# DixianZhu/deBWT

Measured on AMD Instinct MI355X. Metric: Gbp/sec BWT build (30 Gbp synthetic DNA); bit-exact vs CPU ref; 1/2/4/8-GPU, higher is better.
Workload: dtype u64

## Files before the change

### debwt_amd/_lib.py

```python
import ctypes
import os
import subprocess

_HERE = os.path.dirname(os.path.abspath(__file__))
LIB_PATH = os.environ.get("DEBWT_HIP_LIB", os.path.join(_HERE, "libdebwt_hip.so"))
_lib = None


class DebwtConfig(ctypes.Structure):
    _fields_ = [("k", ctypes.c_int), ("device", ctypes.c_int), ("sort_algo", ctypes.c_int),
                ("reserved", ctypes.c_int)]


class DebwtPackedText(ctypes.Structure):
    _fields_ = [("words", ctypes.POINTER(ctypes.c_uint64)), ("nwords", ctypes.c_uint64), ("n", ctypes.c_uint64),
                ("sep", ctypes.POINTER(ctypes.c_uint64)), ("nrec", ctypes.c_uint64),
                ("seconds_read", ctypes.c_double), ("seconds_pack", ctypes.c_double)]


class DebwtStats(ctypes.Structure):
    _fields_ = ([(n, ctypes.c_uint64) for n in (
        "n", "nrec", "red_capacity", "blue_capacity", "blue_bound_num", "case3num", "sp_len",
        "special_branch_num", "n_main", "distinct_keys", "blue_large_blocks", "blue_max_block")] +
        [(n, ctypes.c_float) for n in (
            "ms_extract", "ms_sort", "ms_classify", "ms_sp", "ms_blue", "ms_assemble", "ms_total",
            "ms_host_special")] +
        [("radix_pass_launches", ctypes.c_uint32), ("radix_pass_ms", ctypes.c_float),
         ("radix_pass_keys", ctypes.c_uint64), ("special_path", ctypes.c_uint32), ("special_threads", ctypes.c_uint32),
         ("sort_unfit_stretches", ctypes.c_uint64), ("sort_unfit_network", ctypes.c_uint64),
         ("sort_over_stretches", ctypes.c_uint64), ("sort_bucket_passes", ctypes.c_uint64)])

    def as_dict(self):
        return {n: getattr(self, n) for n, _ in self._fields_}


class DebwtVerifyReport(ctypes.Structure):
    _fields_ = ([(n, ctypes.c_uint64) for n in ("segments", "steps", "mismatches", "broken_links", "search_failures",
                                                "search_steps")] +
                [(n, ctypes.c_float) for n in ("ms_index", "ms_search", "ms_walk")] + [("ok", ctypes.c_int)])

    def as_dict(self):
        return {n: getattr(self, n) for n, _ in self._fields_}


MULTI_STEPS = 24


class DebwtShardReport(ctypes.Structure):
    _fields_ = [("ms", ctypes.c_float * MULTI_STEPS), ("bytes_in", ctypes.c_uint64 * 5), ("bytes_out", ctypes.c_uint64 * 5),
                ("keys", ctypes.c_uint64), ("key_ranges", ctypes.c_uint64), ("blocks", ctypes.c_uint64),
                ("blue_rows", ctypes.c_uint64), ("rows", ctypes.c_uint64), ("bin_lo", ctypes.c_uint32), ("bin_hi", ctypes.c_uint32)]


class DebwtFmInfo(ctypes.Structure):
    _fields_ = ([(n, ctypes.c_uint64) for n in ("n", "nrec", "sa_sample", "samples", "device_bytes")] +
                [("ms_rank", ctypes.c_float), ("ms_samples", ctypes.c_float), ("census", ctypes.c_uint64 * 4)])

    def as_dict(self):
        d = {n: getattr(self, n) for n, _ in self._fields_}
        d["census"] = [int(x) for x in self.census]
        return d


# ... 690 lines not shown
```

### debwt_amd/csrc/debwt_hip.hip

```cpp
#include "../../include/debwt_hip.h"

#include <hip/hip_runtime.h>

#include <algorithm>
#include <new>
#include <chrono>
#include <cmath>
#include <cstdio>
#include <cstring>
#include <atomic>
#include <string>
#include <thread>
#include <tuple>
#include <vector>

#include "radix_sort.h"
#include "special_host.h"
#include "fasta_host.h"
#include "gz_parallel.h"
#include "stage_kernels.h"
#include "special_kernels.h"
#include "verify_kernels.h"
#include "fm_kernels.h"
#include "fm_search_kernels.h"
// ... 804 lines not shown
                    (unsigned long long)r.M, (unsigned long long)in_heavy, (unsigned)RS_BUCKET_HEAVY, (unsigned long long)largest,
                    r.heavy ? "four HBM passes" : "bucket pass");
    }
    return DEBWT_OK;
}

static int sort_begin(debwt_ctx *c) {
    const u64 n = c->n;
    if (c->stage > ST_LOADED) c->stage = ST_LOADED;
    int rc = plan_ranges(c);
    if (rc) return rc;
    u64 maxM = 0;
    for (auto &r : c->ranges) maxM = std::max(maxM, r.M);
    struct ReclaimScope { debwt_ctx *c; ~ReclaimScope() { c->reclaim_ok = false; } } rscope{c};
    c->reclaim_ok = true;
    if (!c->exchange) ENSURE(c, c->keysA, maxM * 8 + 64);
    ENSURE(c, c->keysB, maxM * 8 + 64);
    ENSURE(c, c->rs_skew, (maxM / 2048 + 2) * 4);
    ENSURE(c, c->rs_rle, radix_rle_ws_bytes(maxM));
    if ((rc = heavy_ranges(c))) return rc;
    size_t pair_bytes = 0;
    for (auto &r : c->ranges) {
        const u64 range[2] = {r.key_lo, r.key_hi};
        pair_bytes = std::max(pair_bytes, radix_pair_bytes_u64(r.M, 2 * c->cfg.k, range, r.heavy));
    }
    ENSURE(c, c->rs_pair, pair_bytes);
    ENSURE(c, c->dk, maxM * 8 + 64);
    ENSURE(c, c->dstart, maxM * 4 + 64);
    ENSURE(c, c->pflag, maxM + 64);
    ENSURE(c, c->mchar, c->Mctx + 64);
    c->reclaim_ok = false;
    c->Q = c->B = c->nlarge = 0; c->nfacts_acc = 0; c->n1024 = 0; c->n512 = 0; c->Dsum = 0;
    c->st.sort_unfit_stretches = c->st.sort_unfit_network = c->st.sort_over_stretches = c->st.sort_bucket_passes = 0;
    const size_t P = c->ranges.size();
    HIPCHK(c, hipEventRecord(c->ev[0], c->stream));
    HIPCHK(c, hipEventRecord(c->ev[1], c->stream));
    join_special(c);
    c->special_dev = false;
    if (special_wants_device(c)) {
        if ((rc = special_device_build(c))) return rc;
    } else {
    c->special_running = true;
    c->special_thread = std::thread([c, n]() {
        auto t0 = std::chrono::steady_clock::now();
        build_special_tables(c->h_text, n, c->h_sep.data(), c->nrec, c->K, &c->special);
        c->st.ms_host_special = std::chrono::duration<float, std::milli>(std::chrono::steady_clock::now() - t0).count();
        c->st.special_threads = c->special.threads_used;
        c->st.special_path = c->special.threads_used > 1 ? 1 : 0;
    });
    }
    c->shared_hist = P <= RS_MAX_RANGES && !c->exchange &&
                     (P > 1 || (P == 1 && n >= (1ull << 26) && range_split(c, c->ranges[0]).hbm_shift > 0));
    if (c->shared_hist) {
        const int kb = 2 * c->cfg.k;
        std::vector<u8> rob(SHARD_BINS, 0xFF);
        int shifts[RS_MAX_RANGES];
        for (size_t i = 0; i < P; i++) {
            const u32 lo = (u32)(c->ranges[i].key_lo >> (kb - 12));
            const u32 hi = c->ranges[i].key_hi ? (u32)(c->ranges[i].key_hi >> (kb - 12)) : SHARD_BINS;
            for (u32 b = lo; b < hi; b++) rob[b] = (u8)i;
            shifts[i] = range_split(c, c->ranges[i]).hbm_shift;
        }
        ENSURE(c, c->dest_tab, SHARD_BINS);
        ENSURE(c, c->range_hist, P * radix_text_hist_stride() * sizeof(u32));
        HIPCHK(c, hipMemcpyAsync(c->dest_tab.p, rob.data(), SHARD_BINS, hipMemcpyHostToDevice, c->stream));
        TextKeySrc all{c->text.as<u64>(), c->sepbits.as<u64>(), n, c->K, 0, 0, 0, nullptr, nullptr, 0};
// ... 31 lines not shown
    if (i == 0 && !c->special_dev) {
        join_special(c);
        const SpecialTables &sp = c->special;
        c->nbranch = sp.branch.size();
        ENSURE(c, c->branch, sp.branch.size() * 8 + 64);
        HIPCHK(c, hipMemcpyAsync(c->head_keys.p, sp.head_keys.data(), c->nrec * 8, hipMemcpyHostToDevice, c->stream));
        HIPCHK(c, hipMemcpyAsync(c->spkey.p, sp.key.data(), c->NS * 8, hipMemcpyHostToDevice, c->stream));
        HIPCHK(c, hipMemcpyAsync(c->spchr.p, sp.chr.data(), c->NS, hipMemcpyHostToDevice, c->stream));
        if (!sp.branch.empty())
            HIPCHK(c, hipMemcpyAsync(c->branch.p, sp.branch.data(), sp.branch.size() * 8, hipMemcpyHostToDevice, c->stream));
        if ((rc = special_branch_bitmap(c))) return rc;
    }
    u64 *d_bounds = nullptr;
    {
        const std::vector<uint64_t> &key = c->special.key;
        u64 s0 = 0, s1 = c->NS;
        if ((c->shard_world > 1 || P > 1) && c->special_dev) {
            d_bounds = c->dollar.as<u64>() + 5;
            k_sp_bounds<<<1, 64, 0, c->stream>>>(c->spkey.as<u64>(), c->NS, r.key_lo >> 2, r.key_hi >> 2, d_bounds);
            HIPCHK(c, hipMemcpyAsync(&c->h_scalars[24], d_bounds, 16, hipMemcpyDeviceToHost, c->stream));
        } else if (c->shard_world > 1 || P > 1) {
            s0 = std::lower_bound(key.begin(), key.end(), r.key_lo >> 2) - key.begin();
            s1 = r.key_hi ? (u64)(std::lower_bound(key.begin(), key.end(), r.key_hi >> 2) - key.begin()) : c->NS;
        }
        r.s0 = s0; r.s1 = s1;
    }
    if ((rc = sync_check(c))) return rc;
    if (d_bounds) memcpy(&r.s0, &c->h_scalars[24], 8), memcpy(&r.s1, &c->h_scalars[26], 8);
    c->D = c->h_scalars[0];
    c->Dsum += c->D;
    if (sink.done) {
        c->st.sort_unfit_stretches += c->h_scalars[32]; c->st.sort_unfit_network += c->h_scalars[35];
        c->st.sort_over_stretches += sink.n_over;
    }
    if (r.s1 > r.s0)
        k_special_rows<<<grid_for(r.s1 - r.s0, 256), 256, 0, c->stream>>>(
            c->dk.as<u64>(), c->dstart.as<u32>(), c->D, r.M, c->spkey.as<u64>() + r.s0, r.s1 - r.s0,
            r.Mbase + (r.s0 - c->ranges[0].s0), c->sprow.as<u64>() + r.s0);
    if (P > 1 || c->exchange) {
        if ((rc = classify_local(c))) return rc;
        if ((rc = append_range(c, r))) return rc;
    }
    return DEBWT_OK;
}

static int sort_end(debwt_ctx *c) {
    c->s0 = c->ranges.front().s0; c->s1 = c->ranges.back().s1;
    if (c->ranges.size() > 1 || c->exchange) {
        c->local_done = true;
        HIPCHK(c, hipEventRecord(c->ev[2], c->stream));
        HIPCHK(c, hipEventRecord(c->ev[3], c->stream));
    }
    c->st.distinct_keys = c->Dsum;
    c->st.special_branch_num = c->nbranch;
    c->stage = ST_SORTED;
    return DEBWT_OK;
}

extern "C" int debwt_kmer_sort_rle(debwt_ctx *c) {
    if (!c) return DEBWT_EINVAL;
    if (c->stage < ST_LOADED) return DEBWT_ESTATE;
    if (c->exchange) { c->err = "exchange-mode shard: use debwt_shard_sort_begin/_range/_end"; return DEBWT_ESTATE; }
    HIPCHK(c, hipSetDevice(c->cfg.device));
    int rc = sort_begin(c);
    for (size_t i = 0; !rc && i < c->ranges.size(); i++) rc = sort_range(c, i, nullptr);
    join_special(c);
// ... 6343 lines not shown
```

### debwt_amd/csrc/radix_sort.hip

```cpp
#include "radix_sort.h"

#include <algorithm>
#include <atomic>
#include <cstddef>
#include <utility>
#include <cstdio>
#include <cstdlib>
#include <vector>


template <int FIXED0>
__device__ __forceinline__ u32 rs_digit(const RsDigit &g, u64 k) {
    if (FIXED0 == 2) return __builtin_amdgcn_ubfe((u32)(k >> 32), (u32)g.shift - 32u, (u32)__popc(g.mask));
    if (FIXED0 || g.mode == 0) {
        const u32 lo = (u32)k, hi = (u32)(k >> 32);
        const bool up = g.shift >= 32;
        return __builtin_amdgcn_alignbit(up ? 0u : hi, up ? hi : lo, (u32)g.shift & 31u) & g.mask;
    }
    if (g.mode == 1) return g.tab[(k >> g.tshift) & 4095u];
    u32 q = (u32)(k >> g.tshift), lo = 0, hi = g.nb;
    if (hi <= 16u) {
        for (u32 i = 1; i < hi; i++) lo += g.bounds[i] <= q ? 1u : 0u;
        return lo;
    }
// ... 1526 lines not shown
        for (int r = 0; r < KPT; r++)
            if (cr[r] != 0xFFFFFFFFu) A[RL_PAD(cr[r])] = kk[r];
        __syncthreads();
        if (!tcnt) {
            for (u32 j = tid; j < cnt; j += NT) keys[s + j] = A[RL_PAD(j)];
        } else {
            for (u32 j = tid; j < cnt; j += NT) mchar[s + j] = (u8)(A[RL_PAD(j)] & 3ull);
            u32 hm = 0;
            u64 prev = tid ? A[RL_PAD(tid * KPT - 1)] : 0ull;
#pragma unroll
            for (int r = 0; r < KPT; r++) {
                const u32 j = tid * KPT + (u32)r;
                const u64 key = A[RL_PAD(j)];
                hm |= ((j < cnt && (j == 0 || key != prev)) ? 1u : 0u) << r;
                prev = key;
            }
            const u32 cl = (u32)__popc(hm);
            u32 c;
            u32 o = block_scan_excl(cl, wtmp, &c);
            const bool staged = stg != nullptr && RLT_STAGE_RATIO * c <= cnt;
            if (tid == 0) { tcnt[t] = c | (staged ? RLT_STAGED : 0u); unfit[i] = t | RLU_COUNTED; }
            if (staged) {
                u64 *kd = stg + s;
                unsigned short *id = reinterpret_cast<unsigned short *>(stg + s + c);
#pragma unroll
                for (int r = 0; r < KPT; r++)
                    if ((hm >> r) & 1u) { kd[o] = A[RL_PAD(tid * KPT + r)]; id[o] = (unsigned short)(tid * KPT + r); o++; }
            }
            if (!(staged && drop_sorted))
                for (u32 j = tid; j < cnt; j += NT) keys[s + j] = A[RL_PAD(j)];
        }
    }
}
#endif

__global__ __launch_bounds__(256) void rs_local_unfit_net_kernel(u64 *__restrict__ keys, u64 n, const u64 *__restrict__ bnd,
                                                                 u32 nwtiles, u32 *__restrict__ unfit,
                                                                 const u32 *__restrict__ nunfit, u32 *__restrict__ over,
                                                                 u32 over_cap) {
    constexpr int KPT = 16, NT = 256;
    constexpr u32 CAP = NT * KPT;
    __shared__ u64 A[CAP + CAP / 16];
    const u32 tid = threadIdx.x;
    const u32 nu = nunfit[0];
    if (RLU_CLASSIFY && nunfit[3] == 0) return;
    for (u32 i = blockIdx.x; i < nu; i += gridDim.x) {
        u32 t = unfit[i];
        if (RLU_CLASSIFY) {
            if (!(t & RLU_NET_FLAG)) continue;
            t &= ~RLU_NET_FLAG;
            __syncthreads();
            if (tid == 0) unfit[i] = t;
        }
        const u64 s = bnd[t], e = t + 1 < nwtiles ? bnd[t + 1] : n;
        const u64 cnt64 = e - s;
        __syncthreads();
        if (cnt64 > CAP) {
            if (RLU_CLASSIFY) continue;
            u32 bad = 0;
            for (u64 j = s + tid; j + 1 < e && !bad; j += NT) bad = keys[j] > keys[j + 1] ? 1u : 0u;
            if (__syncthreads_or((int)bad) && tid == 0) {
                const u32 idx = atomicAdd(&over[0], 1u);
                if (idx < over_cap) {
                    u64 *list = reinterpret_cast<u64 *>(over + 4);
                    list[2 * idx] = s; list[2 * idx + 1] = cnt64;
                }
// ... 202 lines not shown
            const u32 m = l_n;
            for (u32 q = 0; q < m; q++) {
                const u32 t = l_t[q];
                const u64 s = l_s[q], e = l_e[q];
                const u32 K = (u32)((e - (u64)t * RLW_H) / RLW_H);
                const u64 k0 = (u64)gy + (W + G - t % G) % G;
                if (k0 >= K) continue;
                const u64 kfirst = keys[s];
                const bool one_run = kfirst == keys[e - 1];
                for (u64 k = k0; k < K; k += G) piece(t, s, e, K, (u32)k, kfirst, one_run);
            }
        }
        return;
    }
    for (u32 i = blockIdx.x; i < nu; i += gridDim.x) {
        const u32 entry = unfit[i];
        const u32 t = RLU_TILE(entry);
        if (entry & RLU_COUNTED) {
            if (!EMIT || ((tcnt[t] & RLT_STAGED) && staging_ok)) continue;
        }
        const u64 s = bnd[t], e = t + 1 < nwtiles ? bnd[t + 1] : n;
        const u64 K64 = (e - (u64)t * RLW_H) / RLW_H;
        const u32 K = (K64 < 1 || (entry & RLU_COUNTED)) ? 1u : (u32)K64;
        if (K >= RLU_LONG) continue;
        const u64 kfirst = keys[s];
        const bool one_run = kfirst == keys[e - 1];
        for (u32 k = 0; k < K; k++) piece(t, s, e, K, k, kfirst, one_run);
    }
}


static size_t rle_nw(u64 n) { return (size_t)(n / RLW_H + 2); }
static size_t rle_nb(u64 n) { return rle_nw(n) / RLT_BLOCK + 2; }
size_t radix_rle_ws_bytes(u64 n) { return 16 + rle_nw(n) * (8 + 12) + rle_nb(n) * 8 + 64; }

__global__ __launch_bounds__(256) void rs_over_move(u64 *__restrict__ keys, u64 *__restrict__ scratch, const u64 *__restrict__ list,
                                                    const u64 *__restrict__ offs, u32 nranges, u64 total, int back,
                                                    const u64 *__restrict__ base = nullptr, int W = 0) {
    const u64 g0 = (u64)blockIdx.x * 1024u;
    if (g0 >= total) return;
    u32 lo = 0, hi = nranges;
    while (lo + 1 < hi) { u32 mid = (lo + hi) >> 1; if (offs[mid] <= g0) lo = mid; else hi = mid; }
    const u64 wmask = W ? (1ull << W) - 1ull : 0ull;
#pragma unroll
    for (int j = 0; j < 4; j++) {
        const u64 g = g0 + (u64)j * 256u + threadIdx.x;
        if (g >= total) break;
        u32 r = lo;
        while (r + 1 < nranges && offs[r + 1] <= g) r++;
        const u64 src = list[2 * r] + (g - offs[r]);
        if (!base) { if (back) keys[src] = scratch[g]; else scratch[g] = keys[src]; }
        else if (back) keys[src] = (scratch[g] & wmask) + base[r];
        else scratch[g] = ((u64)r << W) | (keys[src] - base[r]);
    }
}
__global__ void rs_over_ends(const u64 *__restrict__ keys, const u64 *__restrict__ list, u32 nranges, u64 *__restrict__ ends) {
    const u32 r = blockIdx.x * blockDim.x + threadIdx.x;
    if (r >= nranges) return;
    ends[2 * r] = keys[list[2 * r]];
    ends[2 * r + 1] = keys[list[2 * r] + list[2 * r + 1] - 1];
}

#define RB_NT 256
#define RB_KPT 16
#define RB_CAP (RB_NT * RB_KPT)
#define RB_H (4 * RB_CAP)
#define RB_UNROLL 4
// ... 255 lines not shown
        if (ev) (void)hipEventRecord(pass_events[2 * ev_idx], stream);
        if (aux && strip_last && shift + bits >= hi_bit) {
            dg.out_strip = strip_last;
            rs_scatter_kernel<0, 2, 0><<<nchunks, SC_NT, 0, stream>>>(src, none, dst, n, chunk, dg, ws.counts, digit_tot, nchunks, ctab);
        } else if (aux) rs_scatter_kernel<0, 1, 0><<<nchunks, SC_NT, 0, stream>>>(src, none, dst, n, chunk, dg, ws.counts, digit_tot, nchunks, ctab);
        else if (shift >= 32) rs_scatter_kernel<0, 0, 1><<<nchunks, SC_NT, 0, stream>>>(src, none, dst, n, chunk, dg, ws.counts, digit_tot, nchunks, ctab);
        else rs_scatter_kernel<0, 0, 0><<<nchunks, SC_NT, 0, stream>>>(src, none, dst, n, chunk, dg, ws.counts, digit_tot, nchunks, ctab);
        if (ev) { (void)hipEventRecord(pass_events[2 * ev_idx + 1], stream); ev_idx++; if (npairs) *npairs = ev_idx; }
        derived = pp.nv != 0;
        if (derived) {
            rs_pair_bounds_kernel<<<(nchunks + 1 + 255) / 256, 256, 0, stream>>>(ws.counts, digit_tot, nchunks, pp.rows, n, chunk, nchunks, pair_tab);
            rs_pair_derive_kernel<<<nchunks, RS_RADIX, 0, stream>>>(pair_J, pair_tab, pp.nv, pp.vbase, ws.counts, nchunks);
            rs_pair_launched.fetch_add(1, std::memory_order_relaxed);
        }
        if (final_dst) { src = dst; dst = (npasses - (p + 2)) % 2 == 0 ? final_dst : (src == a ? third : a); }
        else if (third) { src = dst; dst = p + 2 == npasses ? a : (src == b ? third : b); }
        else { u64 *t = src; src = dst; dst = t; }
    }
    return src;
}

size_t radix_text_hist_stride() { return (size_t)RS_RADIX * RS_MAXCHUNKS; }

static int rs_bucket_mode() {
    const char *e = getenv("DEBWT_BUCKET_PASS");
    return !e || !*e ? -1 : (atoi(e) != 0 ? 1 : 0);
}

static int rs_forced_digits() {
    const char *e = getenv("DEBWT_PREFIX_DIGITS");
    const int t = e && *e ? atoi(e) : 0;
    return t >= 1 && t <= 4 ? t : 0;
}
static bool rs_finish_low() {
    const char *e = getenv("DEBWT_FINISH_LOW");
    return !e || !*e || atoi(e) != 0;
}

RadixSplit radix_split(u64 n, int key_bits, int algo, const u64 *range, bool heavy) {
    algo &= 15;
    if (key_bits > 64) key_bits = 64;
    const int mode = rs_bucket_mode();
    int T = 0;
    while ((n >> (8 * T)) > RS_BUCKET_TARGET && T < 4) T++;
    if (mode == 1 && T < 2) T = 2;
    if (rs_forced_digits()) T = rs_forced_digits();
    RadixSplit sp{false, false, 0, 0, 0};
    if (algo != 3 || T == 0 || key_bits - 8 * T < 1) return sp;
    sp.hybrid = true;
    sp.T = T;
    sp.pshift = key_bits - 8 * T;
    const bool ranged = range && (range[0] || range[1]);
    sp.bucket = mode == 1 ? T >= 2 : (mode != 0 && T == 4 && ranged && !heavy);
    sp.hbm_shift = sp.bucket ? sp.pshift + 8 : sp.pshift;
    return sp;
}

static std::atomic<u64> rs_bucket_launched{0};
u64 radix_bucket_passes() { return rs_bucket_launched.load(std::memory_order_relaxed); }
static std::atomic<u64> rs_low_finishes{0};
u64 radix_low_finishes() { return rs_low_finishes.load(std::memory_order_relaxed); }

hipError_t radix_text_hist_ranges(hipStream_t stream, const TextKeySrc &text, const u8 *range_of_bin, int key_bits,
                                  const int *shift, int nranges, u32 *counts) {
    if (nranges < 1 || nranges > RS_MAX_RANGES) return hipErrorInvalidValue;
    u32 nchunks; u64 chunk;
// ... 48 lines not shown
    const bool net_only = (algo & 32) != 0;
    (void)net_only;
    algo &= 15;
    if (key_bits > 64) key_bits = 64;
    if (!text && (n < (rs_bucket_mode() == 1 ? 1u : 2u) || key_bits <= 0)) return a;
    const u64 text_range[2] = {text ? text->key_lo : 0ull, text ? text->key_hi : 0ull};
    if (!key_range && text) key_range = text_range;
    const RadixSplit sp = radix_split(n, key_bits, algo, key_range, heavy);
    if (!sp.hybrid || !ws.over || !ws.h_over) {
        u64 *r = rs_lsd(stream, a, b, n, 0, key_bits, ws, pass_events, max_pairs, npairs, text, aux, 0, nullptr, nullptr, key_range);
        *err = hipGetLastError();
        return r;
    }
    const int pshift = sp.pshift;
    u64 *src = rs_lsd(stream, a, b, n, sp.hbm_shift, key_bits, ws, pass_events, max_pairs, npairs, text, aux, 0, nullptr, nullptr, key_range);
    u64 *other = src == a ? b : a;
    if (sp.bucket && n > 0) {
        const u32 nbt = (u32)((n + RB_H - 1) / RB_H);
        rs_bucket_digit_kernel<<<nbt, RB_NT, 0, stream>>>(src, other, n, sp.hbm_shift, pshift);
        rs_bucket_launched.fetch_add(1, std::memory_order_relaxed);
        u64 *t = src; src = other; other = t;
    }
    const bool low = pshift <= 32 && rs_finish_low();
    if (low) rs_low_finishes.fetch_add(1, std::memory_order_relaxed);
    (void)hipMemsetAsync(ws.over, 0, 16, stream);
    u32 ntiles = (u32)((n + RL_H - 1) / RL_H), nwtiles = (u32)((n + RLW_H - 1) / RLW_H);
    u8 *mark = reinterpret_cast<u8 *>(ws.skew_list);
    (void)hipMemsetAsync(mark, 0, ntiles + 1, stream);
    u32 *rle_ctr = nullptr, *rle_tcnt = nullptr, *rle_unfit = nullptr, *rle_tex = nullptr, *rle_bsum = nullptr, *rle_boff = nullptr;
    u64 *rle_bnd = nullptr;
    if (sink) {
        const size_t nw = rle_nw(n);
        rle_ctr = static_cast<u32 *>(sink->ws);
        rle_bnd = reinterpret_cast<u64 *>(rle_ctr + 4);
        rle_tcnt = reinterpret_cast<u32 *>(rle_bnd + nw);
        rle_unfit = rle_tcnt + nw;
        rle_tex = rle_unfit + nw;
        rle_bsum = rle_tex + nw;
        rle_boff = rle_bsum + rle_nb(n);
        (void)hipMemsetAsync(rle_ctr, 0, 16, stream);
        if (low)
            rs_local_count_kernel<true><<<nwtiles, 64, 0, stream>>>(src, n, pshift, mark, rle_bnd, rle_unfit, rle_ctr, rle_tcnt, sink->mchar,
                                                                    sink->no_staging ? nullptr : other, sink->drop_sorted ? 1 : 0);
        else
            rs_local_count_kernel<false><<<nwtiles, 64, 0, stream>>>(src, n, pshift, mark, rle_bnd, rle_unfit, rle_ctr, rle_tcnt, sink->mchar,
                                                                     sink->no_staging ? nullptr : other, sink->drop_sorted ? 1 : 0);
        const u32 ugrid = nwtiles < 16384u ? nwtiles : 16384u;
#if RLU_CLASSIFY
        u64 *const stg = sink->no_staging ? nullptr : other;
        rs_local_unfit_kernel<8><<<ugrid, 256, 0, stream>>>(src, n, rle_bnd, nwtiles, rle_unfit, rle_ctr, ws.over, ws.over_cap,
                                                            net_only ? 0u : RLU_GAP_MAX, rle_tcnt, sink->mchar, stg, sink->drop_sorted ? 1 : 0);
        rs_local_unfit_kernel<16><<<ugrid < 4096u ? ugrid : 4096u, 256, 0, stream>>>(src, n, rle_bnd, nwtiles, rle_unfit, rle_ctr, ws.over,
                                                                                      ws.over_cap, net_only ? 0u : RLU_GAP_MAX,
                                                                                      rle_tcnt, sink->mchar, stg, sink->drop_sorted ? 1 : 0);
#endif
        rs_local_unfit_net_kernel<<<ugrid, 256, 0, stream>>>(src, n, rle_bnd, nwtiles, rle_unfit, rle_ctr, ws.over, ws.over_cap);
    } else {
        if (low) rs_local_kernel<64, true><<<nwtiles, 64, 0, stream>>>(src, n, pshift, ws.over, ws.over_cap, mark);
        else rs_local_kernel<64><<<nwtiles, 64, 0, stream>>>(src, n, pshift, ws.over, ws.over_cap, mark);
        rs_local_kernel<256><<<ntiles, 256, 0, stream>>>(src, n, pshift, ws.over, ws.over_cap, mark);
    }
    (void)hipMemcpyAsync(ws.h_over, ws.over, 16, hipMemcpyDeviceToHost, stream);
    if ((*err = hipStreamSynchronize(stream)) != hipSuccess) return src;
    u32 nover = ws.h_over[0];
    bool staging_lost = false;
    if (nover) {
        bool whole = nover > ws.over_cap;
        u64 total = 0;
        std::vector<u64> offs, hlist;
        if (!whole) {
            hlist.resize(2 * (size_t)nover);
            (void)hipMemcpyAsync(hlist.data(), ws.over + 4, 16 * (size_t)nover, hipMemcpyDeviceToHost, stream);
            if ((*err = hipStreamSynchronize(stream)) != hipSuccess) return src;
            const u64 *list = hlist.data();
            std::vector<std::pair<u64, u64>> rg(nover);
            for (u32 i = 0; i < nover; i++) rg[i] = {list[2 * i], list[2 * i + 1]};
            std::sort(rg.begin(), rg.end());
            offs.resize(3 * (size_t)nover);
            for (u32 i = 0; i < nover; i++) {
                offs[i] = total; total += rg[i].second;
                offs[nover + 2 * i] = rg[i].first; offs[nover + 2 * i + 1] = rg[i].second;
            }
// ... 39 lines not shown
                    dmax = std::max(dmax, (ends[2 * i + 1] >> pshift) - (ends[2 * i] >> pshift));
                }
                int wb = pshift, rb = 1;
                while (wb < 64 && (dmax >> (wb - pshift))) wb++;
                while ((1ull << rb) < nover) rb++;
                if (wb + rb <= key_bits - 8) {
                    (void)hipMemcpyAsync(d_base, base.data(), 8 * (size_t)nover, hipMemcpyHostToDevice, stream);
                    if ((*err = hipStreamSynchronize(stream)) != hipSuccess) return src;
                    cbase = d_base; W = wb; sort_bits = wb + rb;
                }
            }
            rs_over_move<<<grid, 256, 0, stream>>>(src, scratch, d_list, d_offs, nover, total, 0, cbase, W);
            u64 *r = rs_lsd(stream, scratch, tmp, total, 0, sort_bits, ws, nullptr, 0, nullptr, nullptr, true);
            rs_over_move<<<grid, 256, 0, stream>>>(src, r, d_list, d_offs, nover, total, 1, cbase, W);
            if ((*err = hipStreamSynchronize(stream)) != hipSuccess) return src;
        }
    }
    if (sink) {
        const u32 ug = nwtiles < 2048u ? nwtiles : 2048u;
        const u32 nb = (nwtiles + RLT_BLOCK - 1) / RLT_BLOCK;
        rs_unfit_rle_kernel<0, 0><<<ug, 256, 0, stream>>>(src, n, rle_bnd, nwtiles, rle_unfit, rle_ctr, rle_tcnt, rle_tex,
                                                       rle_boff, sink->dk, sink->dstart, sink->mchar, staging_lost ? 0 : 1);
                rs_unfit_rle_kernel<0, 1><<<dim3(64, RLU_ROWS), RLU_LONG_NT, 0, stream>>>(src, n, rle_bnd, nwtiles, rle_unfit, rle_ctr, rle_tcnt, rle_tex,
                                                       rle_boff, sink->dk, sink->dstart, sink->mchar, staging_lost ? 0 : 1);
        rs_tile_scan1_kernel<<<nb, 256, 0, stream>>>(rle_tcnt, nwtiles, rle_tex, rle_bsum);
        rs_tile_scan2_kernel<<<1, 1024, 0, stream>>>(rle_bsum, nb, rle_boff, rle_ctr + 1);
        rs_tile_emit_kernel<<<(nwtiles + 3) / 4, 256, 0, stream>>>(src, n, rle_bnd, nwtiles, rle_tex, rle_boff, sink->dk, sink->dstart,
                                                                   rle_tcnt, staging_lost ? nullptr : other);
        rs_unfit_rle_kernel<1, 0><<<ug, 256, 0, stream>>>(src, n, rle_bnd, nwtiles, rle_unfit, rle_ctr, rle_tcnt, rle_tex,
                                                       rle_boff, sink->dk, sink->dstart, sink->mchar, staging_lost ? 0 : 1);
                rs_unfit_rle_kernel<1, 1><<<dim3(64, RLU_ROWS), RLU_LONG_NT, 0, stream>>>(src, n, rle_bnd, nwtiles, rle_unfit, rle_ctr, rle_tcnt, rle_tex,
                                                       rle_boff, sink->dk, sink->dstart, sink->mchar, staging_lost ? 0 : 1);
        (void)hipMemcpyAsync(sink->h_total, rle_ctr + 1, sizeof(u32), hipMemcpyDeviceToHost, stream);
        if (sink->h_ctr) (void)hipMemcpyAsync(sink->h_ctr, rle_ctr, 4 * sizeof(u32), hipMemcpyDeviceToHost, stream);
        sink->n_over = nover;
        sink->done = true;
    }
    *err = hipGetLastError();
    return src;
}

hipError_t radix_partition_by_shard(hipStream_t stream, const u64 *src, const TextKeySrc *text, u64 count, u64 *dst,
                                    const RsDigit &dg, u32 nshards, const RadixWorkspace &ws, u64 *offs_host, bool sparse,
                                    u64 capacity) {
    TextKeySrc none{};
    u32 nchunks; u64 chunk;
    rs_plan(count, &nchunks, &chunk);
    u32 *digit_tot = ws.counts + (size_t)RS_RADIX * RS_MAXCHUNKS;
    if (text) {
        TextKeySrc ts = *text;
        rs_hist_kernel<1, 1><<<nchunks, RS_BLOCK, 0, stream>>>(nullptr, ts, count, chunk, dg, ws.counts, nchunks);
    } else {
        rs_hist_kernel<0, 1><<<nchunks, RS_BLOCK, 0, stream>>>(src, none, count, chunk, dg, ws.counts, nchunks);
    }
    rs_scan_digit_kernel<<<RS_RADIX, 1024, 0, stream>>>(ws.counts, nchunks, digit_tot);
    rs_scan_tot_kernel<<<1, RS_RADIX, 0, stream>>>(digit_tot);
    u32 tot[RS_RADIX];
    hipError_t e = hipMemcpyAsync(tot, digit_tot, sizeof tot, hipMemcpyDeviceToHost, stream);
    if (e != hipSuccess) return e;
    if ((e = hipStreamSynchronize(stream)) != hipSuccess) return e;
    for (u32 i = 0; i < nshards; i++) offs_host[i] = tot[i];
    offs_host[nshards] = nshards < RS_RADIX ? tot[nshards] : 0;
    if (offs_host[nshards] > capacity) return hipErrorInvalidValue;
    if (text && sparse) rs_scatter_sparse_kernel<0, 1><<<nchunks, SC_NT, 0, stream>>>(*text, dst, count, chunk, dg, ws.counts, digit_tot, nchunks);
    else if (text) rs_scatter_kernel<1, 1, 0><<<nchunks, SC_NT, 0, stream>>>(nullptr, *text, dst, count, chunk, dg, ws.counts, digit_tot, nchunks);
    else rs_scatter_kernel<0, 1, 0><<<nchunks, SC_NT, 0, stream>>>(src, none, dst, count, chunk, dg, ws.counts, digit_tot, nchunks);
    if ((e = hipStreamSynchronize(stream)) != hipSuccess) return e;
// ... 3 lines not shown
```

### include/debwt_hip.h

```cpp
#ifndef DEBWT_HIP_H
#define DEBWT_HIP_H
#include <stddef.h>
#include <stdint.h>
#ifdef __cplusplus
extern "C" {
#endif

#define DEBWT_OK 0
#define DEBWT_EINVAL (-1)
#define DEBWT_ENOMEM (-2)
#define DEBWT_EDEVICE (-3)
#define DEBWT_ESTATE (-4)
#define DEBWT_ERANGE (-5)
#define DEBWT_EINTERNAL (-6)
#define DEBWT_EIO (-7)

typedef struct debwt_ctx debwt_ctx;

typedef struct {
    int k;
    int device;
    int sort_algo;
    int reserved;
} debwt_config;

typedef struct {
    uint64_t n;
    uint64_t nrec;
    uint64_t red_capacity;
    uint64_t blue_capacity;
    uint64_t blue_bound_num;
    uint64_t case3num;
    uint64_t sp_len;
    uint64_t special_branch_num;
    uint64_t n_main;
    uint64_t distinct_keys;
    uint64_t blue_large_blocks;
    uint64_t blue_max_block;
    float ms_extract, ms_sort, ms_classify, ms_sp, ms_blue, ms_assemble, ms_total, ms_host_special;
    uint32_t radix_pass_launches;
    float radix_pass_ms;
    uint64_t radix_pass_keys;
    uint32_t special_path, special_threads;
    uint64_t sort_unfit_stretches, sort_unfit_network, sort_over_stretches;
    uint64_t sort_bucket_passes;
} debwt_stats;

int debwt_create(const debwt_config *cfg, debwt_ctx **out);
void debwt_destroy(debwt_ctx *ctx);
const char *debwt_strerror(int code);
const char *debwt_last_error(const debwt_ctx *ctx);
int debwt_get_config(const debwt_ctx *ctx, debwt_config *out);

int debwt_load_text(debwt_ctx *ctx, const uint64_t *packed, uint64_t n, const uint64_t *sep, uint64_t nrec);

int debwt_load_ascii(debwt_ctx *ctx, const char *seq, const uint64_t *reclen, uint64_t nrec);

typedef struct {
    uint64_t *words;
    uint64_t nwords;
    uint64_t n;
    uint64_t *sep;
    uint64_t nrec;
    double seconds_read, seconds_pack;
} debwt_packed_text;
int debwt_pack_fasta(const char *path, int threads, debwt_packed_text *out, char *errbuf, size_t errlen);
void debwt_free_packed(debwt_packed_text *p);
int debwt_load_fasta(debwt_ctx *ctx, const char *path, int threads);
#define DEBWT_FASTA_IUPAC_RANDOM 1u
int debwt_pack_fasta_opts(const char *path, int threads, unsigned flags, uint64_t seed, debwt_packed_text *out,
                          char *errbuf, size_t errlen);
int debwt_load_fasta_opts(debwt_ctx *ctx, const char *path, int threads, unsigned flags, uint64_t seed);
uint64_t debwt_fasta_text_bound(const char *path);
void debwt_host_release_hold(int on);

#define DEBWT_RESERVE_ONE_SHOT 1u
#define DEBWT_RESERVE_COMPACT 2u
int debwt_reserve(debwt_ctx *ctx, uint64_t n, uint64_t nrec, double branching, unsigned flags);
// ... 493 lines not shown
```

Measured before the change: 24.39.

## Add wave-level sample-sort split kernel for unfit tiles whose run crosses the tile boundary

Adds a single-wavefront kernel that picks up unfit tiles whose final key group spills past the tile boundary. It sorts a sample in registers with a bitonic network, buckets the low 32-bit words by splitter binary search with LDS atomics, and finishes each small bucket with a rank count. It then writes run heads, mchar and staged keys directly and marks the tile as counted, so the heavier generic unfit kernels can skip it. The kernel is on by default behind an environment switch, adds a split counter to the stats, and grows the workspace header. Tiles whose buckets exceed the gap limit still fall back to the existing path.

```diff
diff --git a/debwt_amd/_lib.py b/debwt_amd/_lib.py
--- a/debwt_amd/_lib.py
+++ b/debwt_amd/_lib.py
@@ -28,7 +28,8 @@
         [("radix_pass_launches", ctypes.c_uint32), ("radix_pass_ms", ctypes.c_float),
          ("radix_pass_keys", ctypes.c_uint64), ("special_path", ctypes.c_uint32), ("special_threads", ctypes.c_uint32),
          ("sort_unfit_stretches", ctypes.c_uint64), ("sort_unfit_network", ctypes.c_uint64),
-         ("sort_over_stretches", ctypes.c_uint64), ("sort_bucket_passes", ctypes.c_uint64)])
+         ("sort_over_stretches", ctypes.c_uint64), ("sort_bucket_passes", ctypes.c_uint64),
+         ("sort_split_stretches", ctypes.c_uint64)])
 
     def as_dict(self):
         return {n: getattr(self, n) for n, _ in self._fields_}
diff --git a/debwt_amd/csrc/debwt_hip.hip b/debwt_amd/csrc/debwt_hip.hip
--- a/debwt_amd/csrc/debwt_hip.hip
+++ b/debwt_amd/csrc/debwt_hip.hip
@@ -860,6 +860,7 @@
     c->reclaim_ok = false;
     c->Q = c->B = c->nlarge = 0; c->nfacts_acc = 0; c->n1024 = 0; c->n512 = 0; c->Dsum = 0;
     c->st.sort_unfit_stretches = c->st.sort_unfit_network = c->st.sort_over_stretches = c->st.sort_bucket_passes = 0;
+    c->st.sort_split_stretches = 0;
     const size_t P = c->ranges.size();
     HIPCHK(c, hipEventRecord(c->ev[0], c->stream));
     HIPCHK(c, hipEventRecord(c->ev[1], c->stream));
@@ -957,6 +958,7 @@
     if (sink.done) {
         c->st.sort_unfit_stretches += c->h_scalars[32]; c->st.sort_unfit_network += c->h_scalars[35];
         c->st.sort_over_stretches += sink.n_over;
+        c->st.sort_split_stretches += c->h_scalars[36];
     }
     if (r.s1 > r.s0)
         k_special_rows<<<grid_for(r.s1 - r.s0, 256), 256, 0, c->stream>>>(
diff --git a/debwt_amd/csrc/radix_sort.hip b/debwt_amd/csrc/radix_sort.hip
--- a/debwt_amd/csrc/radix_sort.hip
+++ b/debwt_amd/csrc/radix_sort.hip
@@ -1582,6 +1582,311 @@
         }
     }
 }
+
+#ifndef RLS_SAMPLE
+#define RLS_SAMPLE 64
+#endif
+#define RLS_CAP 2048u
+static_assert(RLS_SAMPLE == 64 || RLS_SAMPLE == 128 || RLS_SAMPLE == 256, "one, two or four sample values per lane");
+
+__device__ __forceinline__ u32 rls_lane(u32 lane) {
+    asm volatile("" : "+v"(lane));
+    return lane;
+}
+
+__device__ __forceinline__ void rls_sync() {
+    __builtin_amdgcn_fence(__ATOMIC_RELEASE, "wavefront");
+    __builtin_amdgcn_wave_barrier();
+    __builtin_amdgcn_fence(__ATOMIC_ACQUIRE, "wavefront");
+}
+
+template <int V>
+__device__ __forceinline__ void rls_sort_sample(u32 (&x)[V], const u32 lane) {
+    constexpr int LG = 6 + (V == 1 ? 0 : V == 2 ? 1 : 2);
+#pragma unroll
+    for (int lk = 1; lk <= LG; lk++) {
+        const u32 kk = 1u << lk;
+#pragma unroll
+        for (int lj = lk - 1; lj >= 0; lj--) {
+            const int d = 1 << lj;
+            if (d < V) {
+#pragma unroll
+                for (int v = 0; v < V; v++)
+                    if ((v & d) == 0) {
+                        const bool up = ((lane * V + v) & kk) == 0;
+                        const u32 a = x[v], b = x[v | d];
+                        const bool sw = (a > b) == up;
+                        x[v] = sw ? b : a; x[v | d] = sw ? a : b;
+                    }
+            } else {
+                const int dl = d / V;
+                const bool lower = (lane & (u32)dl) == 0;
+#pragma unroll
+                for (int v = 0; v < V; v++) {
+                    const u32 p = (u32)__shfl_xor((int)x[v], dl, 64);
+                    const bool up = ((lane * V + v) & kk) == 0;
+                    const bool pless = p < x[v];
+                    x[v] = ((lower == up) == pless) ? p : x[v];
+                }
+            }
+        }
+    }
+}
+
+__global__ __launch_bounds__(64) __attribute__((amdgpu_waves_per_eu(4, 4)))
+void rs_local_split_kernel(u64 *__restrict__ keys, u64 n, int pshift, const u64 *__restrict__ bnd, u32 nwtiles,
+                           u32 *__restrict__ unfit, const u32 *__restrict__ nunfit, u32 *__restrict__ nsplit, u32 gap_max,
+                           u32 *__restrict__ tcnt, u8 *__restrict__ mchar, u64 *__restrict__ stg, int drop_sorted) {
+    constexpr int KPT = 16, S = RLS_SAMPLE, V = S / 64, WPL = RLS_CAP / 64, CPL = 2 * S / 64;
+    static_assert(RL_PAD(RLW_H) <= RLS_CAP / 2, "the front goes back through the area of the low words");
+    __shared__ u64 A[RLS_CAP / 2];
+    __shared__ u32 spl[S];
+    __shared__ u32 ccnt[2 * S];
+    u32 *const W = reinterpret_cast<u32 *>(A);
+    const u32 lane0 = threadIdx.x;
+    const u32 nu = nunfit[0], G = gridDim.x;
+    const auto entry = [&](const u32 i) -> u32 { return i < nu ? unfit[i] : RLU_NET_FLAG; };
+    const auto bounds = [&](const u32 t, u64 &s, u64 &e) {
+        s = e = 0;
+        if (!(t & (RLU_NET_FLAG | RLU_COUNTED))) { s = bnd[t]; e = t + 1 < nwtiles ? bnd[t + 1] : n; }
+    };
+    u32 t_next = entry(blockIdx.x), t_after = entry(blockIdx.x + G);
+    u64 s_next, e_next;
+    bounds(t_next, s_next, e_next);
+    for (u32 i = blockIdx.x; i < nu; i += G) {
+        const u32 t = t_next;
+        const u64 s = s_next, e = e_next;
+        t_next = t_after;
+        bounds(t_next, s_next, e_next);
+        t_after = i + 2u * G >= i ? entry(i + 2u * G) : RLU_NET_FLAG;
+        if (t & (RLU_NET_FLAG | RLU_COUNTED)) continue;
+        if (e - s > RLW_H - 1u + RLS_CAP) continue;
+        u32 lane = rls_lane(lane0);
+        const u64 x1 = ((u64)t + 1u) * RLW_H;
+        const u64 last = (x1 < n ? x1 : n) - 1u;
+        if (last < s || last >= e || last - s >= RLW_H) continue;
+        constexpr u32 NG = RLW_H / 64;
+        const u64 klast = keys[last];
+        const u64 p = klast >> pshift;
+        const u32 hiw = (u32)(klast >> 32);
+        const u32 span = (u32)(last - s) + 1u;
+        u64 g[NG];
+#pragma unroll
+        for (u32 r = 0; r < NG; r++) g[r] = r * 64u + lane < span ? keys[s + r * 64u + lane] : ~0ull;
+        u32 below = 0;
+#pragma unroll
+        for (u32 r = 0; r < NG; r++) below += (u32)__popcll(__ballot(r * 64u + lane < span && (g[r] >> pshift) != p));
+        const u64 b = s + below;
+        const u32 front = below, L = (u32)(e - b), cnt = front + L;
+        if (front >= RLW_H || L > RLS_CAP) continue;
+        rls_sync();
+        const u32 have = span - front;
+#pragma unroll
+        for (u32 r = 0; r < NG; r++) {
+            const u32 q = r * 64u + lane;
+            if (q >= front && q < span) W[q - front] = (u32)g[r];
+        }
+#pragma unroll
+        for (u32 r = 0; r < WPL; r++)
+            if (have + r * 64u < L) {
+                const u32 j = have + r * 64u + lane;
+                if (j < L) W[j] = (u32)keys[b + j];
+            }
+        rls_sync();
+        u32 w[WPL];
+#pragma unroll
+        for (u32 r = 0; r < WPL; r++) {
+            w[r] = 0xFFFFFFFFu;
+            if (r * 64u < L) {
+                const u32 j = r * 64u + lane;
+                if (j < L) w[r] = W[j];
+            }
+        }
+        u32 bad = 0;
+#pragma unroll
+        for (u32 r = 0; r < WPL; r++)
+            if (r * 64u < L) {
+                const u32 j = r * 64u + lane;
+                if (j + 1u < L) bad |= w[r] > W[j + 1u] ? 1u : 0u;
+            }
+        if (__ballot(bad != 0) != 0ull) {
+            lane = rls_lane(lane0);
+            u32 x[V];
+#pragma unroll
+            for (int v = 0; v < V; v++) x[v] = W[(u32)(((lane * V + v) * L) / S)];
+#pragma unroll
+            for (u32 q = 0; q < CPL; q++) ccnt[q * 64u + lane] = 0;
+            rls_sort_sample<V>(x, lane);
+            const u32 before = (u32)__shfl_up((int)x[V - 1], 1, 64);
+            u32 hmask = 0;
+#pragma unroll
+            for (int v = 0; v < V; v++) {
+                const u32 pv = v ? x[v - 1] : before;
+                hmask |= (((lane == 0 && v == 0) || x[v] != pv) ? 1u : 0u) << v;
+            }
+            const u32 hc = (u32)__popc(hmask), hincl = wave_scan_incl(hc);
+            u32 U = (u32)__shfl((int)hincl, 63, 64);
+            {
+                u32 o = hincl - hc;
+#pragma unroll
+                for (int v = 0; v < V; v++)
+                    if ((hmask >> v) & 1u) { if (o < S - 1u) spl[o] = x[v]; o++; }
+            }
+            if (U > S - 1u) U = S - 1u;
+#pragma unroll
+            for (int v = 0; v < V; v++)
+                if (lane * V + v >= U) spl[lane * V + v] = 0xFFFFFFFFu;
+            rls_sync();
+            u32 cr[WPL];
+#pragma unroll
+            for (u32 r = 0; r < WPL; r++) cr[r] = 0xFFFFFFFFu;
+#pragma unroll
+            for (u32 r0 = 0; r0 < WPL; r0 += 4) {
+                if (r0 * 64u < L) {
+                    u32 lo[4] = {0, 0, 0, 0};
+#pragma unroll
+                    for (u32 step = S / 2; step; step >>= 1)
+#pragma unroll
+                        for (u32 q = 0; q < 4; q++) lo[q] = spl[lo[q] + step - 1u] < w[r0 + q] ? lo[q] + step : lo[q];
+                    u32 at[4];
+#pragma unroll
+                    for (u32 q = 0; q < 4; q++) at[q] = spl[lo[q]];
+#pragma unroll
+                    for (u32 q = 0; q < 4; q++)
+                        if ((r0 + q) * 64u + lane < L) {
+                            const u32 cls = 2u * lo[q] + ((lo[q] < U && at[q] == w[r0 + q]) ? 1u : 0u);
+                            cr[r0 + q] = (cls << 16) | atomicAdd(&ccnt[cls], 1u);
+                        }
+                }
+                __builtin_amdgcn_sched_barrier(0);
+            }
+            rls_sync();
+            u32 cv[CPL], csum = 0, gap = 0;
+#pragma unroll
+            for (u32 q = 0; q < CPL; q++) {
+                cv[q] = ccnt[lane * CPL + q];
+                csum += cv[q];
+                if (!(q & 1u)) gap = cv[q] > gap ? cv[q] : gap;
+            }
+            if (__ballot(gap > gap_max) != 0ull) continue;
+            u32 run = wave_scan_incl(csum) - csum;
+#pragma unroll
+            for (u32 q = 0; q < CPL; q++) { ccnt[lane * CPL + q] = run; run += cv[q]; }
+            rls_sync();
+#pragma unroll
+            for (u32 r = 0; r < WPL; r++)
+                if (cr[r] != 0xFFFFFFFFu) {
+                    const u32 pos = ccnt[cr[r] >> 16] + (cr[r] & 0xFFFFu);
+                    W[pos] = w[r];
+                    cr[r] = (cr[r] & 0xFFFF0000u) | pos;
+                }
+            rls_sync();
+#pragma unroll
+            for (u32 r = 0; r < WPL; r++) {
+                const u32 cls = cr[r] >> 16, pos = cr[r] & 0xFFFFu;
+                u32 np = 0xFFFFFFFFu;
+                if (cr[r] != 0xFFFFFFFFu && !(cls & 1u)) {
+                    const u32 st = ccnt[cls], en = cls + 1u < 2u * S ? ccnt[cls + 1u] : L;
+                    if (en - st > 1) {
+                        const u32 key = w[r];
+                        u32 less = 0;
+                        for (u32 y = st; y < en; y++) {
+                            const u32 ky = W[y];
+                            less += (ky < key || (ky == key && y < pos)) ? 1u : 0u;
+                        }
+                        np = st + less;
+                    }
+                }
+                cr[r] = np;
+                __builtin_amdgcn_sched_barrier(0);
+            }
+            rls_sync();
+#pragma unroll
+            for (u32 r = 0; r < WPL; r++)
+                if (cr[r] != 0xFFFFFFFFu) W[cr[r]] = w[r];
+            rls_sync();
+        }
+        lane = rls_lane(lane0);
+        u64 k[KPT];
+        u32 hm = 0, cl = 0, incl = 0, cf = 0;
+        if (front) {
+#pragma unroll
+            for (int r = 0; r < KPT; r++) k[r] = lane * KPT + r < front ? keys[s + lane * KPT + r] : ~0ull;
+        }
+        u32 cb = 0;
+        for (u32 j0 = 0; j0 < L; j0 += 64u) {
+            const u32 j = j0 + lane;
+            const bool valid = j < L;
+            const u32 wj = valid ? W[j] : 0u;
+            const bool head = valid && (j == 0 || W[j - 1u] != wj);
+            cb += (u32)__popcll(__ballot(head));
+            if (valid) mchar[b + j] = (u8)(wj & 3u);
+        }
+        if (front) {
+            rlw_sort<true>(k, lane);
+            const u64 before = __shfl_up(k[KPT - 1], 1, 64);
+#pragma unroll
+            for (int r = 0; r < KPT; r++) {
+                const u64 pk = r ? k[r - 1] : before;
+                hm |= ((lane * KPT + r < front && ((lane == 0 && r == 0) || k[r] != pk)) ? 1u : 0u) << r;
+            }
+            cl = (u32)__popc(hm); incl = wave_scan_incl(cl);
+            cf = (u32)__shfl((int)incl, 63, 64);
+        }
+        lane = rls_lane(lane0);
+        const u32 c = cf + cb;
+        const bool staged = stg != nullptr && RLT_STAGE_RATIO * c <= cnt;
+        if (lane == 0) { tcnt[t] = c | (staged ? RLT_STAGED : 0u); unfit[i] = t | RLU_COUNTED; atomicAdd(nsplit, 1u); }
+        u64 *kd = stg + s;
+        unsigned short *id = reinterpret_cast<unsigned short *>(stg + s + c);
+        if (staged) {
+            u32 o = cf;
+            for (u32 j0 = 0; j0 < L; j0 += 64u) {
+                const u32 j = j0 + lane;
+                const bool valid = j < L;
+                const u32 wj = valid ? W[j] : 0u;
+                const bool head = valid && (j == 0 || W[j - 1u] != wj);
+                const u64 bm = __ballot(head);
+                if (head) {
+                    const u32 oo = o + (u32)__popcll(bm & lanemask_lt());
+                    kd[oo] = ((u64)hiw << 32) | wj; id[oo] = (unsigned short)(front + j);
+                }
+                o += (u32)__popcll(bm);
+            }
+        }
+        const bool back = !(staged && drop_sorted);
+        if (back)
+            for (u32 j = lane; j < L; j += 64u) keys[b + j] = ((u64)hiw << 32) | W[j];
+        if (front) {
+            if (staged) {
+                u32 o = incl - cl;
+#pragma unroll
+                for (int r = 0; r < KPT; r++)
+                    if ((hm >> r) & 1u) { kd[o] = k[r]; id[o] = (unsigned short)(lane * KPT + r); o++; }
+            }
+            if (lane * KPT < front) {
+                u8 *dst = mchar + s + lane * KPT;
+                if (lane * KPT + KPT <= front) {
+                    u32 wv[4] = {0, 0, 0, 0};
+#pragma unroll
+                    for (int r = 0; r < KPT; r++) wv[r >> 2] |= ((u32)k[r] & 3u) << (8 * (r & 3));
+                    __builtin_memcpy(dst, wv, 16);
+                } else {
+#pragma unroll
+                    for (int r = 0; r < KPT; r++) if (lane * KPT + r < front) dst[r] = (u8)(k[r] & 3ull);
+                }
+            }
+            if (back) {
+                rls_sync();
+#pragma unroll
+                for (int r = 0; r < KPT; r++)
+                    if (lane * KPT + r < front) A[RL_PAD(lane * KPT + r)] = k[r];
+                rls_sync();
+                for (u32 j = lane; j < front; j += 64u) keys[s + j] = A[RL_PAD(j)];
+            }
+        }
+    }
+}
 #endif
 
 __global__ __launch_bounds__(256) void rs_local_unfit_net_kernel(u64 *__restrict__ keys, u64 n, const u64 *__restrict__ bnd,
@@ -1850,7 +2155,7 @@
 
 static size_t rle_nw(u64 n) { return (size_t)(n / RLW_H + 2); }
 static size_t rle_nb(u64 n) { return rle_nw(n) / RLT_BLOCK + 2; }
-size_t radix_rle_ws_bytes(u64 n) { return 16 + rle_nw(n) * (8 + 12) + rle_nb(n) * 8 + 64; }
+size_t radix_rle_ws_bytes(u64 n) { return 32 + rle_nw(n) * (8 + 12) + rle_nb(n) * 8 + 64; }
 
 __global__ __launch_bounds__(256) void rs_over_move(u64 *__restrict__ keys, u64 *__restrict__ scratch, const u64 *__restrict__ list,
                                                     const u64 *__restrict__ offs, u32 nranges, u64 total, int back,
@@ -2172,6 +2477,10 @@
     const int t = e && *e ? atoi(e) : 0;
     return t >= 1 && t <= 4 ? t : 0;
 }
+static bool rs_finish_split() {
+    const char *e = getenv("DEBWT_FINISH_SPLIT");
+    return !e || !*e || atoi(e) != 0;
+}
 static bool rs_finish_low() {
     const char *e = getenv("DEBWT_FINISH_LOW");
     return !e || !*e || atoi(e) != 0;
@@ -2286,13 +2595,13 @@
     if (sink) {
         const size_t nw = rle_nw(n);
         rle_ctr = static_cast<u32 *>(sink->ws);
-        rle_bnd = reinterpret_cast<u64 *>(rle_ctr + 4);
+        rle_bnd = reinterpret_cast<u64 *>(rle_ctr + 8);
         rle_tcnt = reinterpret_cast<u32 *>(rle_bnd + nw);
         rle_unfit = rle_tcnt + nw;
         rle_tex = rle_unfit + nw;
         rle_bsum = rle_tex + nw;
         rle_boff = rle_bsum + rle_nb(n);
-        (void)hipMemsetAsync(rle_ctr, 0, 16, stream);
+        (void)hipMemsetAsync(rle_ctr, 0, 32, stream);
         if (low)
             rs_local_count_kernel<true><<<nwtiles, 64, 0, stream>>>(src, n, pshift, mark, rle_bnd, rle_unfit, rle_ctr, rle_tcnt, sink->mchar,
                                                                     sink->no_staging ? nullptr : other, sink->drop_sorted ? 1 : 0);
@@ -2302,6 +2611,10 @@
         const u32 ugrid = nwtiles < 16384u ? nwtiles : 16384u;
 #if RLU_CLASSIFY
         u64 *const stg = sink->no_staging ? nullptr : other;
+        if (low && !net_only && rs_finish_split())
+            rs_local_split_kernel<<<nwtiles < 32768u ? nwtiles : 32768u, 64, 0, stream>>>(src, n, pshift, rle_bnd, nwtiles, rle_unfit, rle_ctr,
+                                                                                         rle_ctr + 4, RLU_GAP_MAX, rle_tcnt, sink->mchar, stg,
+                                                                                         sink->drop_sorted ? 1 : 0);
         rs_local_unfit_kernel<8><<<ugrid, 256, 0, stream>>>(src, n, rle_bnd, nwtiles, rle_unfit, rle_ctr, ws.over, ws.over_cap,
                                                             net_only ? 0u : RLU_GAP_MAX, rle_tcnt, sink->mchar, stg, sink->drop_sorted ? 1 : 0);
         rs_local_unfit_kernel<16><<<ugrid < 4096u ? ugrid : 4096u, 256, 0, stream>>>(src, n, rle_bnd, nwtiles, rle_unfit, rle_ctr, ws.over,
@@ -2407,7 +2720,7 @@
                 rs_unfit_rle_kernel<1, 1><<<dim3(64, RLU_ROWS), RLU_LONG_NT, 0, stream>>>(src, n, rle_bnd, nwtiles, rle_unfit, rle_ctr, rle_tcnt, rle_tex,
                                                        rle_boff, sink->dk, sink->dstart, sink->mchar, staging_lost ? 0 : 1);
         (void)hipMemcpyAsync(sink->h_total, rle_ctr + 1, sizeof(u32), hipMemcpyDeviceToHost, stream);
-        if (sink->h_ctr) (void)hipMemcpyAsync(sink->h_ctr, rle_ctr, 4 * sizeof(u32), hipMemcpyDeviceToHost, stream);
+        if (sink->h_ctr) (void)hipMemcpyAsync(sink->h_ctr, rle_ctr, 5 * sizeof(u32), hipMemcpyDeviceToHost, stream);
         sink->n_over = nover;
         sink->done = true;
     }
diff --git a/include/debwt_hip.h b/include/debwt_hip.h
--- a/include/debwt_hip.h
+++ b/include/debwt_hip.h
@@ -44,6 +44,7 @@
     uint32_t special_path, special_threads;
     uint64_t sort_unfit_stretches, sort_unfit_network, sort_over_stretches;
     uint64_t sort_bucket_passes;
+    uint64_t sort_split_stretches;
 } debwt_stats;
 
 int debwt_create(const debwt_config *cfg, debwt_ctx **out);
```

Result: no change. 24.41, median of 4 (+0.1%).
